# Jamy-L/Handheld-Multi-Frame-Super-Resolution

Measured on AMD Instinct MI355X. Metric: output Mpix/s for 12MP x 20-frame x2 SR burst; max-abs diff vs reference, higher is better.
Workload: dtype f32

## Files before the change

### handheld-multi-frame-super-resolution_amd/csrc/hhsr_robustness.hip

```cpp
#include "hhsr_common.h"

__device__ __forceinline__ double dodgson(double x) {
    const double a = fabs(x);
    if (a <= 0.5) return -2.0 * a * a + 1.0;
    if (a <= 1.5) return a * a - 5.0 / 2.0 * a + 1.5;
    return 0.0;
}

template <int NC>
__device__ __forceinline__ bool dodgson_sample(const float* __restrict__ LR, int lh, int lw, int y, int x, double fx,
                                               double fy, float out[NC]) {
    const double ly = ((double)y + fy + 0.5) / 2.0 - 0.5;
    const double lx = ((double)x + fx + 0.5) / 2.0 - 0.5;
    if (!(ly >= 0.0 && ly < (double)lh && lx >= 0.0 && lx < (double)lw)) return false;
    const int cy = (int)rint(ly), cx = (int)rint(lx);
    const size_t plane = (size_t)lh * lw;
    float b[NC];
#pragma unroll
    for (int c = 0; c < NC; ++c) b[c] = 0.f;
    double wacc = 0.0;
#pragma unroll
    for (int i = -1; i <= 1; ++i) {
        const int y_ = clampi(cy + i, 0, lh - 1);
        const double wy = dodgson((double)y_ - ly);
// ... 209 lines not shown
    const bool inb = dodgson_sample<3>(cm, lh, lw, y, x, (double)f.x, (double)f.y, cmu);
    if (!inb) cmu[0] = cmu[1] = cmu[2] = INFINITY;
    const size_t plane = (size_t)H * W, o = (size_t)y * W + x;
    double d_sq = 0.0;
#pragma unroll
    for (int c = 0; c < 3; ++c) {
        const float b = rmean[c * plane + o];
        const float dp = fabsf(b - cmu[c]);
        int id = 0;
        const double bb = 1000.0 * (double)b;
        if (isfinite(bb)) id = clampi((int)rint(bb), 0, ncurve - 1);
        const double d_t = difc[id];
        const float dp2f = dp * dp;
        const double dp2 = (double)dp2f;
        const double shrink = dp2 / (dp2 + d_t * d_t);
        d_sq += dp2 * shrink * shrink;
    }
    const float dsf = (float)d_sq, ssf = ssq[o];
    const float e = expf(-dsf / ssf);
    double v = (double)(S[(size_t)tiy * nx + tix] * e) - t;
    v = v > 0.0 ? v : 0.0;
    v = v < 1.0 ? v : 1.0;
    R[o] = (float)v;
}

constexpr int RF_T = 16;
constexpr int RF_BX = 32, RF_BY = 32;
constexpr int RF_WN = 11;

struct RobAxis {
    int fi;
    float h;
    bool lt, eq;
    bool ok;
};
__device__ __forceinline__ RobAxis rob_axis(float f) {
    const double fd = (double)f, fl = floor(fd), ff = fd - fl;
    RobAxis a;
    a.ok = fabs(fd) < 1.0e9;
    a.fi = a.ok ? (int)fl : 0;
    a.h = (float)(0.5 * ff);
    a.lt = ff < 0.5;
    a.eq = ff == 0.5;
    return a;
}
__device__ __forceinline__ bool rob_centre(const RobAxis& a, int p, int len, int& c, float& r) {
    const int n = p + a.fi, m = n >> 1, odd = n & 1;
    const bool up = odd && !a.lt && (!a.eq || (m & 1));
    c = m + (up ? 1 : 0);
    const float base = odd ? 0.25f + a.h : a.h - 0.25f;
    r = (up ? 1.0f : 0.0f) - base;
    return a.ok && (n >= 1 || (n == 0 && !a.lt)) && (n < 2 * len || (n == 2 * len && a.lt));
}
__device__ __forceinline__ void dodgson3(float r, int c, int len, float w[3]) {
    const float inner = fmaf(-2.0f * r, r, 1.0f);
    const float am = fabsf(r - 1.0f), ap = fabsf(r + 1.0f);
    const float om = fmaf(am, am, fmaf(-2.5f, am, 1.5f)), op = fmaf(ap, ap, fmaf(-2.5f, ap, 1.5f));
    w[0] = c - 1 >= 0 ? om : inner;
    w[1] = inner;
    w[2] = c + 1 <= len - 1 ? op : inner;
}

__device__ __forceinline__ void rob_row4(const float (*win)[RF_WN][RF_WN + 2], const RobAxis& ay, const RobAxis& ax,
                                         int wy0, int wx0, int y, int x0, int lh, int lw, const float rbk[4][3],
                                         const float d_t2[4][3], const float iss[4], float Sv, float tf, float out[4]) {
    int cy;
    float ry, wyv[3];
    const bool iny = rob_centre(ay, y, lh, cy, ry);
    dodgson3(ry, cy, lh, wyv);
    const int wi0 = cy - 1 - wy0;
    float cmu[4][3];
#pragma unroll
    for (int ph = 0; ph < 2; ++ph) {
        int cx;
        float rx;
        const bool inx = rob_centre(ax, x0 + ph, lw, cx, rx);
#pragma unroll
        for (int c = 0; c < 3; ++c) cmu[ph][c] = cmu[ph + 2][c] = INFINITY;
        if (iny && inx && cx >= 1 && cx + 2 <= lw - 1) {
            float wxv[3], w[3][3], wacc = 0.f;
            dodgson3(rx, cx, lw, wxv);
#pragma unroll
            for (int i = 0; i < 3; ++i)
#pragma unroll
                for (int j = 0; j < 3; ++j) {
                    w[i][j] = wyv[i] * wxv[j];
                    wacc += w[i][j];
                }
            const float iw = __builtin_amdgcn_rcpf(wacc);
            const int wj0 = cx - 1 - wx0;
#pragma unroll
            for (int c = 0; c < 3; ++c) {
                float g4[3][4];
#pragma unroll
                for (int i = 0; i < 3; ++i)
#pragma unroll
                    for (int j = 0; j < 4; ++j) g4[i][j] = win[c][wi0 + i][wj0 + j];
#pragma unroll
                for (int q = 0; q < 2; ++q) {
                    float b = 0.f;
#pragma unroll
                    for (int i = 0; i < 3; ++i)
#pragma unroll
                        for (int j = 0; j < 3; ++j) b = fmaf(g4[i][j + q], w[i][j], b);
                    cmu[ph + 2 * q][c] = b * iw;
                }
            }
        } else {
            int cx2;
            float rx2;
            const bool inx2 = rob_centre(ax, x0 + ph + 2, lw, cx2, rx2);
#pragma unroll
            for (int q = 0; q < 2; ++q) {
                const int cxq = q ? cx2 : cx;
                const float rxq = q ? rx2 : rx;
                if (iny && (q ? inx2 : inx)) {
                    float wxv[3], b0 = 0.f, b1 = 0.f, b2 = 0.f, wacc = 0.f;
                    dodgson3(rxq, cxq, lw, wxv);
                    const int wj0 = cxq - 1 - wx0;
#pragma unroll
                    for (int i = 0; i < 3; ++i) {
#pragma unroll
                        for (int j = 0; j < 3; ++j) {
                            const float w = wyv[i] * wxv[j];
                            b0 = fmaf(win[0][wi0 + i][wj0 + j], w, b0);
                            b1 = fmaf(win[1][wi0 + i][wj0 + j], w, b1);
                            b2 = fmaf(win[2][wi0 + i][wj0 + j], w, b2);
                            wacc += w;
                        }
                    }
                    const float iw = __builtin_amdgcn_rcpf(wacc);
                    cmu[ph + 2 * q][0] = b0 * iw;
                    cmu[ph + 2 * q][1] = b1 * iw;
                    cmu[ph + 2 * q][2] = b2 * iw;
                }
            }
        }
    }
#pragma unroll
    for (int k = 0; k < 4; ++k) {
        float d_sq = 0.f;
#pragma unroll
        for (int c = 0; c < 3; ++c) {
            const float dp = fabsf(rbk[k][c] - cmu[k][c]);
            const float dp2 = dp * dp;
            const float shrink = dp2 * __builtin_amdgcn_rcpf(dp2 + d_t2[k][c]);
            d_sq += dp2 * shrink * shrink;
        }
        const float e = __builtin_amdgcn_exp2f((-d_sq * iss[k]) * 1.44269504088896341f);
        out[k] = __builtin_amdgcn_fmed3f(Sv * e - tf, 0.f, 1.f);
    }
}

constexpr int ROB_GROUP = 4;
struct RobGroup {
    const float* cm[ROB_GROUP];
    const float2* flow[ROB_GROUP];
    const float* S[ROB_GROUP];
    float* R[ROB_GROUP];
    int n;
};

template <bool VEC, typename V, typename T>
__device__ __forceinline__ V rob_load4(const T* __restrict__ p, int x0, int W) {
    if constexpr (VEC) {
        return *reinterpret_cast<const V*>(p);
    } else {
        V v;
        v.x = x0 < W ? p[0] : T(0);
        v.y = x0 + 1 < W ? p[1] : T(0);
        v.z = x0 + 2 < W ? p[2] : T(0);
        v.w = x0 + 3 < W ? p[3] : T(0);
        return v;
    }
}
template <bool VEC>
__device__ __forceinline__ void rob_store4(float* __restrict__ p, const float out[4], int x0, int W) {
    if constexpr (VEC) {
        *reinterpret_cast<float4*>(p) = make_float4(out[0], out[1], out[2], out[3]);
    } else {
#pragma unroll
        for (int q = 0; q < 4; ++q)
            if (x0 + q < W) p[q] = out[q];
    }
}

template <bool VEC>
__global__ void __launch_bounds__(256) k_rob_frames_row4(RobGroup gq, int lh, int lw, const float* __restrict__ rmean,
                                                          const float* __restrict__ ssq,
                                                          const uint32_t* __restrict__ cidx, int ny, int nx, int ts,
                                                          const double* __restrict__ difc, double t, int H, int W,
                                                          double Mt2, float s1, float s2, int rows_lo, int rows_hi) {
    __shared__ float s_g[2][2][3][RF_WN][RF_WN + 2];
    __shared__ float4 s_tab[ROB_GROUP][2][2][2];
    const int lx4 = threadIdx.x & 7, ly_ = threadIdx.x >> 3;
    const int grp = lx4 >> 2, v = ly_ >> 4;
    const int bid = xcd_remap(blockIdx.y * gridDim.x + blockIdx.x, gridDim.x * gridDim.y);
    const int bxi = bid % gridDim.x, byi = bid / gridDim.x;
    const int x0 = bxi * RF_BX + 4 * lx4, y = byi * RF_BY + ly_;
    const size_t gplane = (size_t)lh * lw, plane = (size_t)H * W;
    const int tg = (ly_ & (RF_T - 1)) * 4 + (lx4 & 3);
    constexpr int WSZ = 3 * RF_WN * RF_WN, NST = (WSZ + 63) / 64;
    const bool live = x0 < W && y < H;
    const size_t o = live ? (size_t)y * W + x0 : 0;
    float4 rb4[3];
#pragma unroll
    for (int c = 0; c < 3; ++c) rb4[c] = rob_load4<VEC, float4>(rmean + c * plane + o, x0, W);
    const float4 ss4 = rob_load4<VEC, float4>(ssq + o, x0, W);
    const uint4 ci4 = rob_load4<VEC, uint4>(cidx + o, x0, W);
    const float rbk[4][3] = {{rb4[0].x, rb4[1].x, rb4[2].x}, {rb4[0].y, rb4[1].y, rb4[2].y},
                             {rb4[0].z, rb4[1].z, rb4[2].z}, {rb4[0].w, rb4[1].w, rb4[2].w}};
    const float ssk[4] = {ss4.x, ss4.y, ss4.z, ss4.w};
    const uint32_t cik[4] = {ci4.x, ci4.y, ci4.z, ci4.w};
    float d_t2[4][3], iss[4];
#pragma unroll
    for (int k = 0; k < 4; ++k) {
#pragma unroll
        for (int c = 0; c < 3; ++c) {
            const float d = (float)difc[(cik[k] >> (10 * c)) & 1023u];
            d_t2[k][c] = d * d;
        }
        iss[k] = __builtin_amdgcn_rcpf(ssk[k]);
    }
    if (threadIdx.x < gq.n * 4) {
        const int fr = threadIdx.x >> 2, vv = (threadIdx.x >> 1) & 1, gg = threadIdx.x & 1;
        const int tsx0 = bxi * RF_BX + gg * RF_T, tsy0 = byi * RF_BY + vv * RF_T;
        const size_t tl = (size_t)(min(tsy0, H - 1) / ts) * nx + min(tsx0, W - 1) / ts;
        const float2 f = gq.flow[fr][tl];
        const RobAxis ay = rob_axis(f.y), ax = rob_axis(f.x);
        int wy0, wx0;
        float r_;
        rob_centre(ay, tsy0, lh, wy0, r_);
        rob_centre(ax, tsx0, lw, wx0, r_);
        wy0 = clampi(wy0, -4, lh + 4) - 1;
        wx0 = clampi(wx0, -4, lw + 4) - 1;
        const int flags = (ay.lt ? 1 : 0) | (ay.eq ? 2 : 0) | (ay.ok ? 4 : 0) | (ax.lt ? 8 : 0) | (ax.eq ? 16 : 0) | (ax.ok ? 32 : 0);
        s_tab[fr][vv][gg][0] = make_float4(__int_as_float(ay.fi), ay.h, __int_as_float(wy0), __int_as_float(flags));
        float Sv;
        if (gq.S[fr]) {
            Sv = gq.S[fr][tl];
        } else {
            const int tiy = (int)(tl / nx), tix = (int)(tl - (size_t)tiy * nx);
            float mnx = INFINITY, mny = INFINITY, mxx = -INFINITY, mxy = -INFINITY;
            for (int i = -1; i <= 1; ++i)
                for (int j = -1; j <= 1; ++j) {
                    const int yy = tiy + i, xx = tix + j;
                    if (yy >= -rows_lo && yy < ny + rows_hi && xx >= 0 && xx < nx) {
                        const float2 q = gq.flow[fr][(ptrdiff_t)yy * nx + xx];
                        mxx = fmaxf(mxx, q.x); mxy = fmaxf(mxy, q.y);
                        mnx = fminf(mnx, q.x); mny = fminf(mny, q.y);
                    }
                }
            const float d0 = mxx - mnx, d1 = mxy - mny;
            const float m = d0 * d0 + d1 * d1;
            Sv = ((double)m > Mt2) ? s1 : s2;
        }
        s_tab[fr][vv][gg][1] = make_float4(__int_as_float(ax.fi), ax.h, __int_as_float(wx0), Sv);
    }
    __syncthreads();
    float st[NST];
    int fci[NST];
    unsigned fco[NST];
#pragma unroll
    for (int u = 0; u < NST; ++u) {
        const int p = tg + 64 * u;
        const int c = p / (RF_WN * RF_WN), q = p - c * (RF_WN * RF_WN);
        const int i = q / RF_WN, j = q - i * RF_WN;
        fci[u] = (i << 8) | j;
        fco[u] = (unsigned)c * (unsigned)gplane;
    }
    auto fetch = [&](int fr) {
        const float* __restrict__ cm = gq.cm[fr];
        const int wy0 = __float_as_int(s_tab[fr][v][grp][0].z), wx0 = __float_as_int(s_tab[fr][v][grp][1].z);
#pragma unroll
        for (int u = 0; u < NST; ++u) {
            const int p = tg + 64 * u;
            if (p < WSZ) {
                const int gy = clampi(wy0 + (fci[u] >> 8), 0, lh - 1), gx = clampi(wx0 + (fci[u] & 255), 0, lw - 1);
                const unsigned off = (fco[u] + (unsigned)(__mul24(gy, lw) + gx)) * 4u;
                st[u] = *reinterpret_cast<const float*>(reinterpret_cast<const char*>(cm) + off);
            }
        }
    };
    if (gq.n > 0) fetch(0);
    for (int fr = 0; fr < gq.n; ++fr) {
        const float4 t0 = s_tab[fr][v][grp][0], t1 = s_tab[fr][v][grp][1];
        const int flags = __float_as_int(t0.w);
        RobAxis ay, ax;
        ay.fi = __float_as_int(t0.x); ay.h = t0.y; ay.lt = flags & 1; ay.eq = flags & 2; ay.ok = flags & 4;
        ax.fi = __float_as_int(t1.x); ax.h = t1.y; ax.lt = flags & 8; ax.eq = flags & 16; ax.ok = flags & 32;
        const int wy0 = __float_as_int(t0.z), wx0 = __float_as_int(t1.z);
        const float Sv = t1.w;
        if (fr) __syncthreads();
#pragma unroll
        for (int u = 0; u < NST; ++u) {
            const int p = tg + 64 * u;
            if (p < WSZ) {
                const int c = p / (RF_WN * RF_WN), q = p - c * (RF_WN * RF_WN);
                const int i = q / RF_WN, j = q - i * RF_WN;
                s_g[grp][v][c][i][j] = st[u];
            }
        }
        __syncthreads();
        if (fr + 1 < gq.n) fetch(fr + 1);
        if (!live) continue;
        float out[4];
        rob_row4(s_g[grp][v], ay, ax, wy0, wx0, y, x0, lh, lw, rbk, d_t2, iss, Sv, (float)t, out);
        rob_store4<VEC>(gq.R[fr] + o, out, x0, W);
    }
}

static bool rob_grouped(int ts, const uint32_t* ref_curve_index, int ncurve) {
    return ts % RF_T == 0 && ref_curve_index && ncurve <= 1024;
}

static void rob_frames_launch(const float* const* comp_means, int n_frames, int lh, int lw, const float* ref_means,
                              const float* ref_sigma_sq, const uint32_t* ref_curve_index, const float* const* flows, int ny,
                              int nx, int ts, const float* const* S, double Mt, float s1, float s2, const double* diff_curve,
                              double t, float* const* R, int flow_rows_before, int flow_rows_after, hipStream_t stream) {
    const int H = 2 * lh, W = 2 * lw;
    bool vec = W % 4 == 0 && (((uintptr_t)ref_means | (uintptr_t)ref_sigma_sq | (uintptr_t)ref_curve_index) & 15) == 0;
    for (int n = 0; n < n_frames; ++n) vec = vec && ((uintptr_t)R[n] & 15) == 0;
    for (int n0 = 0; n0 < n_frames; n0 += ROB_GROUP) {
        RobGroup g;
        g.n = n_frames - n0 < ROB_GROUP ? n_frames - n0 : ROB_GROUP;
        for (int k = 0; k < ROB_GROUP; ++k) {
            const int n = n0 + (k < g.n ? k : 0);
            g.cm[k] = comp_means[n];
            g.flow[k] = reinterpret_cast<const float2*>(flows[n]);
            g.S[k] = S ? S[n] : nullptr;
            g.R[k] = R[n];
        }
        hipLaunchKernelGGL(vec ? k_rob_frames_row4<true> : k_rob_frames_row4<false>,
                           dim3(hhsr_cdiv(W, RF_BX), hhsr_cdiv(H, RF_BY)), dim3(256), 0, stream, g, lh, lw, ref_means,
                           ref_sigma_sq, ref_curve_index, ny, nx, ts, diff_curve, t, H, W, Mt * Mt, s1, s2, flow_rows_before,
                           flow_rows_after);
    }
}

extern "C" int hhsr_rob_frame(const float* comp_means, int lh, int lw, const float* ref_means,
                              const float* ref_sigma_sq, const uint32_t* ref_curve_index, const float* flow, int ny,
                              int nx, int ts, const float* S, const double* diff_curve, int ncurve, double t, float* R,
                              void* stream) {
    HHSR_ARG(comp_means && ref_means && ref_sigma_sq && flow && S && diff_curve && R);
    HHSR_ARG(lh > 0 && lw > 0 && ts > 0 && ncurve > 0);
    const int H = 2 * lh, W = 2 * lw;
    HHSR_ARG(ny * ts >= H && nx * ts >= W);
    if (rob_grouped(ts, ref_curve_index, ncurve))
        rob_frames_launch(&comp_means, 1, lh, lw, ref_means, ref_sigma_sq, ref_curve_index, &flow, ny, nx, ts, &S, 0.0, 0.f,
                          0.f, diff_curve, t, &R, 0, 0, (hipStream_t)stream);
    else
        hipLaunchKernelGGL(k_rob_frame, dim3(hhsr_cdiv(W, 64), hhsr_cdiv(H, 4)), dim3(256), 0, (hipStream_t)stream,
                           comp_means, lh, lw, ref_means, ref_sigma_sq, reinterpret_cast<const float2*>(flow), nx, ts,
                           S, diff_curve, ncurve, t, R, H, W);
    HHSR_LAUNCHED();
}

extern "C" int hhsr_rob_frames(const float* const* comp_means, int n_frames, int lh, int lw, const float* ref_means,
                               const float* ref_sigma_sq, const uint32_t* ref_curve_index, const float* const* flows,
                               int ny, int nx, int ts, const float* const* S, double Mt, float s1, float s2,
                               const double* diff_curve, int ncurve, double t, float* const* R, int flow_rows_before,
                               int flow_rows_after, void* stream) {
    HHSR_ARG(comp_means && flows && R && n_frames >= 0 && flow_rows_before >= 0 && flow_rows_after >= 0);
    for (int n = 0; n < n_frames; ++n) HHSR_ARG(comp_means[n] && flows[n] && (!S || S[n]) && R[n]);
    HHSR_ARG(ref_means && ref_sigma_sq && diff_curve && lh > 0 && lw > 0 && ts > 0 && ncurve > 0);
    const int H = 2 * lh, W = 2 * lw;
    HHSR_ARG(ny * ts >= H && nx * ts >= W);
    if (!rob_grouped(ts, ref_curve_index, ncurve)) {
        if (!S) {
            hhsr_set_error("hhsr_rob_frames: S = NULL (weights evaluated inside the kernel) needs the grouped kernel: "
                           "ts %% 16 == 0, packed curve indices");
            return -3;
        }
        for (int n = 0; n < n_frames; ++n) {
            const int rc = hhsr_rob_frame(comp_means[n], lh, lw, ref_means, ref_sigma_sq, ref_curve_index, flows[n], ny, nx,
                                          ts, S[n], diff_curve, ncurve, t, R[n], stream);
            if (rc) return rc;
        }
        return 0;
    }
    rob_frames_launch(comp_means, n_frames, lh, lw, ref_means, ref_sigma_sq, ref_curve_index, flows, ny, nx, ts, S, Mt, s1, s2,
                      diff_curve, t, R, flow_rows_before, flow_rows_after, (hipStream_t)stream);
    HHSR_LAUNCHED();
}

constexpr int LM_TX = 64, LM_TY = 16;

__global__ void __launch_bounds__(256) k_local_min5(const float* __restrict__ R, int H, int W,
                                                     float* __restrict__ r, float* __restrict__ acc) {
    __shared__ float s[LM_TY + 4][LM_TX + 4 + 1];
    __shared__ float s_row[LM_TY + 4][LM_TX + 1];
    const int x0 = blockIdx.x * LM_TX, y0 = blockIdx.y * LM_TY;
    for (int p = threadIdx.x; p < (LM_TY + 4) * (LM_TX + 4); p += 256) {
        const int i = p / (LM_TX + 4), j = p - i * (LM_TX + 4);
        s[i][j] = R[(size_t)clampi(y0 + i - 2, 0, H - 1) * W + clampi(x0 + j - 2, 0, W - 1)];
    }
    __syncthreads();
    for (int p = threadIdx.x; p < (LM_TY + 4) * LM_TX; p += 256) {
        const int i = p / LM_TX, j = p - i * LM_TX;
        float m = s[i][j];
#pragma unroll
        for (int k = 1; k < 5; ++k) m = fminf(m, s[i][j + k]);
        s_row[i][j] = m;
    }
    __syncthreads();
    for (int p = threadIdx.x; p < LM_TY * LM_TX; p += 256) {
        const int i = p / LM_TX, j = p - i * LM_TX;
        const int y = y0 + i, x = x0 + j;
        if (y < H && x < W) {
            float m = s_row[i][j];
#pragma unroll
            for (int k = 1; k < 5; ++k) m = fminf(m, s_row[i + k][j]);
            r[(size_t)y * W + x] = m;
            if (acc) acc[(size_t)y * W + x] += m;
        }
    }
}

extern "C" int hhsr_local_min5(const float* R, int H, int W, float* r, float* acc_r, void* stream) {
    HHSR_ARG(R && r && H > 0 && W > 0 && R != r);
    hipLaunchKernelGGL(k_local_min5, dim3(hhsr_cdiv(W, LM_TX), hhsr_cdiv(H, LM_TY)), dim3(256), 0,
                       (hipStream_t)stream, R, H, W, r, acc_r);
    HHSR_LAUNCHED();
}

struct RobSumFrames {
    const float* r[HHSR_MAX_FRAMES];
    int n;
};

__global__ void __launch_bounds__(256) k_rob_sum(RobSumFrames fr, size_t count, int load, double mfc, float m32, float below,
                                                  float above, double* __restrict__ sum64, float* __restrict__ mask32,
                                                  float* __restrict__ dec32) {
    const size_t i = (size_t)blockIdx.x * 256 + threadIdx.x;
    if (i >= count) return;
    double s = load ? sum64[i] : 0.0;
    for (int n = 0; n < fr.n; ++n) s += (double)fr.r[n][i];
    if (sum64) sum64[i] = s;
    float a = (float)s;
    if (mask32) mask32[i] = a;
    if (dec32) {
        if (s < mfc && a >= m32) a = below;
        if (s > mfc && a <= m32) a = above;
        dec32[i] = a;
    }
}

__global__ void __launch_bounds__(256) k_rob_sum_min5(RobSumFrames fr, int H, int W, int load, double mfc, float m32,
                                                       float below, float above, double* __restrict__ sum64,
                                                       float* __restrict__ mask32, float* __restrict__ dec32) {
    __shared__ float s[LM_TY + 4][LM_TX + 4 + 1];
    __shared__ float s_row[LM_TY + 4][LM_TX + 1];
    constexpr int NIN = ((LM_TY + 4) * (LM_TX + 4) + 255) / 256, NROW = (LM_TY + 4) * LM_TX / 256, NOUT = LM_TY * LM_TX / 256;
    const int x0 = blockIdx.x * LM_TX, y0 = blockIdx.y * LM_TY, tid = threadIdx.x;
    unsigned off[NIN];
#pragma unroll
    for (int u = 0; u < NIN; ++u) {
        const int p = tid + 256 * u, i = p / (LM_TX + 4), j = p - i * (LM_TX + 4);
        off[u] = (unsigned)(clampi(y0 + i - 2, 0, H - 1) * W + clampi(x0 + j - 2, 0, W - 1));
    }
    double acc[NOUT];
#pragma unroll
    for (int u = 0; u < NOUT; ++u) {
        const int p = tid + 256 * u, i = p / LM_TX, j = p - i * LM_TX;
        const bool live = y0 + i < H && x0 + j < W;
        acc[u] = (load && live) ? sum64[(size_t)(y0 + i) * W + x0 + j] : 0.0;
    }
    float pre[NIN];
    auto fetch = [&](int n) {
#pragma unroll
        for (int u = 0; u < NIN; ++u)
            if (tid + 256 * u < (LM_TY + 4) * (LM_TX + 4)) pre[u] = fr.r[n][off[u]];
    };
    if (fr.n > 0) fetch(0);
    for (int n = 0; n < fr.n; ++n) {
#pragma unroll
        for (int u = 0; u < NIN; ++u) {
            const int p = tid + 256 * u, i = p / (LM_TX + 4), j = p - i * (LM_TX + 4);
            if (p < (LM_TY + 4) * (LM_TX + 4)) s[i][j] = pre[u];
// ... 255 lines not shown
```

### handheld-multi-frame-super-resolution_amd/handheld_super_resolution/config.py

```python
from __future__ import annotations

import copy
from typing import Any, Mapping

__all__ = ["Config", "OmegaConf", "DEFAULTS", "default_config", "HIP_KNOBS", "hip_opt"]


class Config(dict):

    def __init__(self, data: Mapping | None = None, **kw):
        super().__init__()
        if data:
            for k, v in dict(data).items():
                self[k] = v
        for k, v in kw.items():
            self[k] = v

    @staticmethod
    def _wrap(v: Any) -> Any:
        if isinstance(v, Config):
            return v
        if isinstance(v, Mapping):
            return Config(v)
        if isinstance(v, tuple):
# ... 51 lines not shown
            raise AttributeError(k) from None

    def get(self, k, default=None):
        return self[k] if k in self else default

    def update(self, other=(), **kw):
        for k, v in dict(other, **kw).items():
            self[k] = v

    def copy(self):
        return Config(copy.deepcopy(dict(self)))

    def __deepcopy__(self, memo):
        return Config({k: copy.deepcopy(v, memo) for k, v in self.items()})


def _to_container(c):
    if isinstance(c, Mapping):
        return {k: _to_container(v) for k, v in c.items()}
    if isinstance(c, (list, tuple)):
        return [_to_container(v) for v in c]
    return c


def _merge_into(dst: Config, src: Mapping):
    for k, v in src.items():
        if isinstance(v, Mapping) and isinstance(dst.get(k), Mapping):
            _merge_into(dst[k], v)
        else:
            dst[k] = copy.deepcopy(v)


class OmegaConf:

    @staticmethod
    def create(obj=None):
        return Config(obj or {})

    @staticmethod
    def load(path):
        import yaml

        with open(path, "r") as f:
            return Config(yaml.safe_load(f) or {})

    @staticmethod
    def merge(*configs):
        out = Config()
        for c in configs:
            _merge_into(out, c)
        return out

    @staticmethod
    def to_container(cfg, resolve=True):
        return _to_container(cfg)

    @staticmethod
    def from_dotlist(items):
        import yaml

        out = Config()
        for it in items:
            key, _, val = it.partition("=")
            node = out
            parts = key.split(".")
            for p in parts[:-1]:
                if p not in node:
                    node[p] = {}
                node = node[p]
            node[parts[-1]] = yaml.safe_load(val)
        return out


DEFAULTS = {
    "scale": 1,
    "mode": "bayer",
    "debug": False,
    "verbose": 1,
    "grey_method": "FFT",
    "noise_model": {"alpha": None, "beta": None},
    "block_matching": {
        "tuning": {
            "factors": [1, 2, 4, 4],
            "tile_size": "SNR_based",
            "tile_size_factors": [1, 1, 1, 0.5],
            "search_radii": [1, 4, 4, 4],
            "metrics": ["L1", "L2", "L2", "L2"],
            "flow_upscale_mode": "nearest",
        }
    },
    "ica": {"tuning": {"n_iter": 3, "sigma_blur": 0}},
    "robustness": {
        "enabled": True,
        "save_mask": True,
        "tuning": {"t": 0.12, "s1": 2, "s2": 12, "Mt": 0.8},
    },
    "merging": {
        "kernel": "steerable",
        "selection_law": "linear",
        "tuning": {
            "k_detail": "SNR_based",
            "k_denoise": "SNR_based",
            "D_th": "SNR_based",
            "D_tr": "SNR_based",
            "k_stretch": 4,
            "k_shrink": 2,
        },
    },
    "postprocessing": {
        "enabled": True,
        "do_color_correction": False,
        "do_gamma_correction": True,
        "do_tonemapping": False,
        "sharpening": {"enabled": True, "amount": 1.5, "radius": 3},
        "do_devignetting": False,
    },
    "accumulated_robustness_denoiser": {
        "median": {"enabled": False, "radius_max": 3, "max_frame_count": 8},
        "gauss": {"enabled": False, "sigma_max": 1.5, "max_frame_count": 8},
        "merge": {"enabled": False, "rad_max": 2, "max_multiplier": 8, "max_frame_count": 2},
    },
    "compat": {
        "ica64_row_bug": True,
    },
}


def default_config(**overrides) -> Config:
    cfg = Config(copy.deepcopy(DEFAULTS))
    if overrides:
        _merge_into(cfg, overrides)
    return cfg


HIP_KNOBS = {
    "graph": True,
    "batch": True,
    "fused_merge": True,
    "fused_align": True,
    "weight_fp64": False,
    "merge_kernel": "auto",
    "strategy": "rows",
    "stage_frames": 0,
    "chunk": None,
    "streams": None,
    "merge_chain": None,
    "merge_link_after": None,
    "host_chunk_sizes": None,
    "inject_flows": None,
    "raw_norm": None,
    "max_flow": None,
    "align_cost": None,
}


def hip_opt(config, name):
    default = HIP_KNOBS[name]
    hip = config.get("hip", None) if hasattr(config, "get") else None
    return default if hip is None else hip.get(name, default)
```

### handheld-multi-frame-super-resolution_amd/handheld_super_resolution/super_resolution.py

```python
import atexit
import os
import threading
import time

import numpy as np
import torch

from . import _lib
from .config import hip_opt
from .utils_image import compute_grey_images, compute_grey_images_batch
from .utils import divide, add, getTime, timer
from .alignment import init_alignment, build_gaussian_pyramids, align_batch, can_align_batch
from .params import sanitize_config, update_snr_config
from .robustness import (init_robustness, compute_robustness, compute_robustness_group, noise_curves_to_device, RobustnessSum,
                         ref_planes, upscale_warp_stats, mono_sigma_sq)
from .kernels import estimate_kernels, frame_stats, frame_stats_batch
from .merge import merge, merge_ref, merge_burst, can_fuse_acc_r, merge_fusions


def denoiser_enabled(config, store=True):
    den = config.accumulated_robustness_denoiser
    if "enabled" in den:
        return bool(den.enabled)
    on = bool(den.median.enabled or den.gauss.enabled or den.merge.enabled)
    if store:
        den.enabled = on
    return on


def accumulation(config):
    denoiser_on = denoiser_enabled(config)
    return denoiser_on, denoiser_on or bool(config.robustness.save_mask)


def main_plan(config, shape, n_comp, denoiser_on, accumulate_r):
    fused_merge = bool(hip_opt(config, "fused_merge"))
    quiet = not (config.verbose >= 1 or bool(config.debug))
    fused = fused_merge and not denoiser_on
    den_fused = fused_merge and denoiser_on and can_fuse_acc_r(config) and n_comp > 0 and quiet
    batch = (fused and quiet) or den_fused
    fuse_acc, fuse_min = merge_fusions(config, shape, n_comp, accumulate_r and not den_fused, denoiser_on)
    return fused, batch, fused and fuse_acc, batch and fuse_min, den_fused


def _device():
    if not torch.cuda.is_available():
        raise RuntimeError("handheld_super_resolution (MI355X build): no HIP device is visible; this package has no "
                           "CPU path (the NumPy oracle under oracle/ is test infrastructure only)")
    return torch.device("cuda", torch.cuda.current_device())


ROB_GROUP = 4


def front_groups(k, batch, given, robustness, mono, batchable):
    whole = k >= 2 and batch and ((given == k and robustness and not mono) or (given == 0 and batchable))
    return [k] if whole else [1] * k


def _tensors(x):
    if torch.is_tensor(x):
        yield x
    elif isinstance(x, (tuple, list)):
        for y in x:
            yield from _tensors(y)


DEFAULT_STREAMS = 2
LARGE_FRAME = 40_000_000
_stream_pool = {}


class _Staged:
    __slots__ = ("tensor", "event")

    def __init__(self, tensor, event):
        self.tensor, self.event = tensor, event


_upload_streams = {}


_LATE_FORK = os.environ.get("HHSR_LATE_FORK") is not None


class BurstPipeline:

    def __init__(self, config, device=None):
        self.config = config
        self.device = device or _device()
        self.mono = config.mode != "bayer"
        self.cfa = [[int(v) for v in row] for row in config.exif.cfa_pattern]
        self.wb = [float(v) for v in config.exif.white_balance]
        self.curves = noise_curves_to_device(config.noise_model.std_curve, config.noise_model.diff_curve, self.device)
        self.grey_method = config.grey_method
        self.ref = None
        self._streams = _stream_pool.setdefault(self.device.index, [])
        self._inject_flows = hip_opt(config, "inject_flows")
        self._raw_norm = hip_opt(config, "raw_norm")
        self.flow_rows = (0, 0)
        self.ref_wait = True
        self._batch = bool(hip_opt(config, "batch")) and (self.mono or self.grey_method == "FFT") and config.verbose < 2

    def _ingest(self, img):
        staged = isinstance(img, _Staged)
        if staged:
            if img.event is not None:
                cur = torch.cuda.current_stream(self.device)
                cur.wait_event(img.event)
                img.tensor.record_stream(cur)
            img = img.tensor
        t = img if torch.is_tensor(img) else torch.as_tensor(img)
        if t.dtype.is_floating_point:
            return _lib.f32c(t, self.device)
        if (t.is_cuda and not staged) or self._raw_norm is None:
            raise ValueError("integer frames are sensor counts: give config.hip.raw_norm = {black_levels, white_level} "
                             "(host arrays), or pass normalised float frames")
        from .utils_dng import normalize_burst, normalize_packed, packed_width

        width = packed_width(self._raw_norm, t)
        if width is not None:
            return normalize_packed(t, width, self._raw_norm["packing"], self._raw_norm["black_levels"],
                                    self._raw_norm["white_level"], self.wb, self.cfa, device=self.device)
        return normalize_burst(t, self._raw_norm["black_levels"], self._raw_norm["white_level"], self.wb, self.cfa,
                               device=self.device)

    def prefetch(self, imgs):
        out, stream = [], None
        for img in imgs:
            t = img if torch.is_tensor(img) else (torch.as_tensor(img) if isinstance(img, np.ndarray) else None)
            if t is None or t.is_cuda or not t.is_pinned():
                out.append(img)
                continue
            if stream is None:
                stream = _upload_streams.get(self.device.index)
                if stream is None:
                    from .graph import shared_streams

                    stream = _upload_streams[self.device.index] = shared_streams(self.device)[1]
            if t.dtype == torch.float64:
                t = t.to(torch.float32).pin_memory()
            with torch.cuda.stream(stream):
                d = t.contiguous().to(self.device, non_blocking=True)
                ev = torch.cuda.Event()
                ev.record(stream)
            self._last_upload = ev
            out.append(_Staged(d, ev))
        return out

    def uploads_done(self):
        ev = getattr(self, "_last_upload", None)
        if ev is not None:
            ev.synchronize()
            self._last_upload = None

    def _timed(self, func, level, start_s=None, end_s=None):
        return timer(func, self.config.verbose >= level, start_s, end_s)

    def init_ref(self, ref_img, alignment=True, robustness=True):
        with torch.cuda.device(self.device):
            return self._init_ref(ref_img, alignment, robustness)

    def _init_ref(self, ref_img, alignment, robustness):
        cfg = self.config
        main = torch.cuda.current_stream(self.device)
        self._entry = torch.cuda.Event()
        self._entry.record(main)
        self._entry_fresh = True
        self.ref = self._ingest(ref_img)
        self.align_state = self.grey_ref = None
        if alignment:
            sanitize_config(cfg, tuple(self.ref.shape))
            grey = self.ref if self.mono else self._timed(
                compute_grey_images, 3, end_s="- Ref grey image estimated by {}".format(self.grey_method))(
                self.ref, self.grey_method)
            self.align_state = self._timed(init_alignment, 2, "\nInitializing alignment", "Alignment initialized (Total)")(
                grey, cfg)
            self.grey_ref = grey
        self._align_ready = torch.cuda.Event()
        self._align_ready.record(main)
        self.ref_means = self.ref_vars = self.ref_covs = self.ref_sigma_sq = None
        if robustness and cfg.robustness.enabled and self.mono:
            m, v, self.ref_covs = self._timed(frame_stats, 2, "\nEstimating ref image local stats + kernels",
                                              "Local stats + kernels estimated (Total)")(
                self.ref, self.cfa, self.wb, cfg, want_vars=True)
            self.ref_means, self.ref_vars = upscale_warp_stats(m), upscale_warp_stats(v)
            self.ref_sigma_sq = mono_sigma_sq(self.ref_means, self.ref_vars, self.curves[0])
        elif robustness and cfg.robustness.enabled:
            m, v, self.ref_covs = self._timed(frame_stats, 2, "\nEstimating ref image local stats + kernels",
                                              "Local stats + kernels estimated (Total)")(
                self.ref, self.cfa, self.wb, cfg, want_vars=True)
            self.ref_means, self.ref_sigma_sq = ref_planes(m, v, self.curves[0])
            self.ref_vars = None
        elif robustness:
            self.ref_means, self.ref_vars = init_robustness(self.ref, self.cfa, self.wb, cfg)
            self.ref_covs = estimate_kernels(self.ref, cfg)
        self._ref_ready = torch.cuda.Event()
        self._ref_ready.record(main)
        return self

    def flow_grid(self):
        lvl0 = self.align_state[0][-1]
        ts = int(self.config.block_matching.tuning.tile_size)
        return lvl0.shape[0] // ts, lvl0.shape[1] // ts

    def align_frames(self, comp_imgs, n_streams=None):
        with torch.cuda.device(self.device):
            comp_imgs = self.prefetch([comp_imgs[i] for i in range(len(comp_imgs))])
            chunks = self._chunks(len(comp_imgs), n_streams)
            out = self._on_streams(len(chunks), n_streams, False,
                                   lambda ci, wait: self._grouped(comp_imgs, wait, chunks[ci], None, stats=False))
            return [f for chunk in out for f in chunk]

    def _grouped(self, imgs, wait_ref, indices, flows, stats=True):
        fl = [None if flows is None else flows[i] for i in indices]
        groups = front_groups(len(indices), self._batch, sum(f is not None for f in fl), bool(self.config.robustness.enabled),
                              self.mono, can_align_batch(self.config))
        out, i0 = [], 0
        for k in groups:
            out += self._front_group([imgs[i] for i in indices[i0:i0 + k]], wait_ref, fl[i0:i0 + k], stats)
            i0 += k
        return out

    def _front_group(self, imgs, wait_ref, flows, stats=True):
        cfg = self.config
        raws = [self._ingest(img) for img in imgs]
        if flows[0] is not None:
            flows = [_lib.f32c(f, self.device) for f in flows]
        else:
            greys = raws if self.mono else self._timed(
                compute_grey_images_batch, 3, end_s="- grey images estimated by {}".format(self.grey_method))(raws, self.grey_method)
            pyramids = build_gaussian_pyramids(greys, cfg.block_matching.tuning.factors)
            if wait_ref is not None:
                torch.cuda.current_stream(self.device).wait_event(self._align_ready)
            st = self.align_state
            flows = self._timed(align_batch, 2, "\nBeginning alignment", "Image aligned (Total)")(
                st[0], st[5], pyramids, cfg, st[3], st[4])
        if not stats:
            return flows
        if not cfg.robustness.enabled:
            est = self._timed(estimate_kernels, 2, "\nEstimating kernels", "Kernels estimated (Total)")
            return [(raw, f, est(raw, cfg), None) for raw, f in zip(raws, flows)]
        stat = self._timed(frame_stats if self.mono else frame_stats_batch, 2, "\nEstimating kernels + guide statistics",
                           "Kernels + guide statistics estimated (Total)")
        sts = [stat(raw, self.cfa, self.wb, cfg) for raw in raws] if self.mono else stat(raws, self.cfa, self.wb, cfg)
        return [(raw, f, st[2], st[0]) for raw, f, st in zip(raws, flows, sts)]

    def _robustness(self, fronts, accumulate_r=None, fuse_local_min=False):
        cfg = self.config
        if not cfg.robustness.enabled or len(fronts) == 1 or self.mono:
            rob = self._timed(compute_robustness, 2, "\nEstimating robustness", "Robustness estimated (Total)")
            return [(raw, flow, covs,
                     rob(raw, self.ref_means, self.ref_vars, flow, self.cfa, self.wb, self.curves, cfg,
                                        accumulate_into=accumulate_r, ref_sigma_sq=self.ref_sigma_sq, comp_means=means,
                                        fuse_local_min=fuse_local_min and cfg.robustness.enabled,
                                        flow_rows=self.flow_rows))
                    for raw, flow, covs, means in fronts]
        rs = compute_robustness_group([f[0] for f in fronts], self.ref_means, [f[1] for f in fronts], self.curves, cfg,
                                      self.ref_sigma_sq, [f[3] for f in fronts], accumulate_into=accumulate_r,
                                      fuse_local_min=fuse_local_min, flow_rows=self.flow_rows)
        return [(f[0], f[1], f[2], r) for f, r in zip(fronts, rs)]

    def process_frame(self, img, accumulate_r=None, wait_ref=None, fuse_local_min=False, index=None, flow=None):
        if flow is None and self._inject_flows is not None and index is not None:
            flow = self._inject_flows[index]
        fronts = self._front_group([img], wait_ref, [flow])
        if wait_ref is not None:
            torch.cuda.current_stream(self.device).wait_event(wait_ref)
        return self._robustness(fronts, accumulate_r, fuse_local_min)[0]

    def process_frames(self, comp_imgs, accumulate_r=None, n_streams=None, fuse_local_min=False, flows=None):
        with torch.cuda.device(self.device):
            n = len(comp_imgs)
            comp_imgs = self.prefetch(comp_imgs)
            chunks = self._chunks(n, n_streams)
            if flows is None:
                flows = self._inject_flows

            def work(ci, wait):
                fronts = self._grouped(comp_imgs, wait, chunks[ci], flows)
                if wait is not None:
                    torch.cuda.current_stream(self.device).wait_event(wait)
                return self._robustness(fronts, accumulate_r if wait is None else None, fuse_local_min)

            out = self._on_streams(len(chunks), n_streams, accumulate_r is not None, work)
            return [f for chunk in out for f in chunk]

    def _chunks(self, n, n_streams=None):
        streams = self._n_streams(n_streams)
        size = self._chunk_size()
        n_chunks = min(n, streams * -(-n // (streams * size))) if n else 0
        chunks, i = [], 0
        for c in range(n_chunks):
            k = n // n_chunks + (1 if c < n % n_chunks else 0)
            chunks.append(list(range(i, i + k)))
            i += k
        return chunks

    def _chunk_size(self):
        chunk = hip_opt(self.config, "chunk")
        return max(1, min(ROB_GROUP if chunk is None else int(chunk), _lib.MAX_BATCH))

    def _n_streams(self, n_streams):
        if n_streams is None:
            n_streams = hip_opt(self.config, "streams")
        if n_streams is None:
            n_streams = 1 if self.ref is not None and self.ref.numel() >= LARGE_FRAME else DEFAULT_STREAMS
        return max(1, int(n_streams))

    def _on_streams(self, n, n_streams, serial, work):
        n_streams = self._n_streams(n_streams)
        early = bool(self.ref_wait and getattr(self, "_entry_fresh", False) and n_streams > 1 and not serial and n >= 1
                     and not _LATE_FORK)
        self._entry_fresh = False
        if not early and (n_streams <= 1 or serial or n < 2):
            return [work(i, None) for i in range(n)]
        main = torch.cuda.current_stream(self.device)
        if len(self._streams) < n_streams:
            self._streams += [torch.cuda.Stream(self.device) for _ in range(n_streams - len(self._streams))]
        pool = self._streams[:n_streams]
        entry = torch.cuda.Event()
        entry.record(main)
        for s in pool:
            s.wait_event(self._entry if early else entry)
        results = []
        for i in range(n):
            s = pool[i % n_streams]
            with torch.cuda.stream(s):
                f = work(i, entry if early else (self._ref_ready if self.ref_wait else None))
            for t in _tensors(f):
                t.record_stream(main)
            results.append(f)
        for s in pool:
            main.wait_stream(s)
        return results

    def output_size(self):
        s = self.config.scale
        H, W = self.ref.shape
        return round(s * H), round(s * W)


_main_runners = []
_main_runners_lock = threading.Lock()


def _drop_host_runners():
    while _main_runners:
        _, _, runner = _main_runners.pop()
        runner.close()


atexit.register(_drop_host_runners)


def _host_runner(config, device):
    from .graph import ConfigWatch, HostBurstRunner

    with _main_runners_lock:
        for k, (cfg, watch, runner) in enumerate(_main_runners):
            if cfg is config and runner.device == device:
                _main_runners.append(_main_runners.pop(k))
                if watch.changed(config):
                    _main_runners.pop()
                    break
                return runner
        watch = ConfigWatch()
        watch.changed(config)
        runner = HostBurstRunner(config, device)
        _main_runners.append((config, watch, runner))
        while len(_main_runners) > 2:
            _main_runners.pop(0)[2].close()
        return runner


def main(ref_img, comp_imgs, config, *, _no_runner=False):
    if not _no_runner and torch.cuda.is_available():
        from .graph import HostBurstRunner

        denoiser_enabled(config)
        if HostBurstRunner.usable(config, ref_img, comp_imgs):
            return _host_runner(config, _device()).call_cloned(ref_img, comp_imgs)
    verbose = config.verbose >= 1
    debug_mode = bool(config.debug)
    debug_dict = {"robustness": [], "flow": []}
    denoiser_on, accumulate_r = accumulation(config)

    if verbose:
        torch.cuda.synchronize()
        t1 = time.perf_counter()
        print("\nProcessing reference image ---------\n")
    pipe = BurstPipeline(config).init_ref(ref_img)
    dev = pipe.device
    H, W = pipe.ref.shape
    sH, sW = pipe.output_size()
    fused, batch, fuse_acc, fuse_min, den_fused = main_plan(config, (H, W), len(comp_imgs), denoiser_on, accumulate_r)
    acc_sum = RobustnessSum((H, W), dev) if denoiser_on else None
    accumulated_r = torch.zeros((H, W), dtype=torch.float32, device=dev) if (accumulate_r and not denoiser_on) else None
    num = torch.empty((sH, sW, 3), dtype=torch.float32, device=dev)
    den = None
    if den_fused:
        den = torch.empty_like(num)
    elif not fused:
        num.zero_()
        den = torch.zeros_like(num)
    if verbose:
        torch.cuda.synchronize()
        getTime(t1, "\nRef Img processed (Total)")

    frames = []
    n_images = len(comp_imgs)
    if batch:
        frames = pipe.process_frames([comp_imgs[i] for i in range(n_images)], None if fuse_acc else accumulated_r,
                                     fuse_local_min=fuse_min)
        if den_fused:
            acc_sum.add_many([f[3] for f in frames], unfiltered=fuse_min)
        n_images = 0
    for im_id in range(n_images):
        if verbose:
            torch.cuda.synchronize()
            print("\nProcessing image {} ---------\n".format(im_id + 1))
            im_time = time.perf_counter()
        raw, flow, covs, r = pipe.process_frame(comp_imgs[im_id], None if fuse_acc else accumulated_r, index=im_id)
        if acc_sum is not None:
            acc_sum.add(r)
        if fused:
            frames.append((raw, flow, covs, r))
        else:
            pipe._timed(merge, 2, "\nAccumulating Image", "Image accumulated (Total)")(raw, flow, covs, r, num, den, pipe.cfa,
                                                                                          config)
        if debug_mode:
            debug_dict["flow"].append(flow.cpu().numpy())
            debug_dict["robustness"].append(r.cpu().numpy())
        if verbose:
            torch.cuda.synchronize()
            getTime(im_time, "\nImage processed (Total)")

    ref_covs = pipe.ref_covs
    if fused:
        pipe._timed(merge_burst, 2, "\nAccumulating all frames + ref Img + normalising", "Burst merged (Total)")(
            frames, pipe.ref, ref_covs, num, None, pipe.cfa, config, do_ref=True, divide=True,
            acc_r=accumulated_r if fuse_acc else None, local_min=fuse_min)
    else:
        if den_fused:
            merge_burst(frames, None, None, num, den, pipe.cfa, config, do_ref=False, divide=False, store_den=True,
                        local_min=fuse_min)
        dec = acc_sum.for_decisions(config.accumulated_robustness_denoiser.merge.max_frame_count) if denoiser_on else None
        if den_fused:
            merge_ref(pipe.ref, ref_covs, num, den, pipe.cfa, config, dec, divide=True, fast=True)
        else:
            pipe._timed(merge_ref, 2, "\nAccumulating ref Img", "Ref Img accumulated (Total)")(
                pipe.ref, ref_covs, num, den, pipe.cfa, config, dec)
            pipe._timed(divide, 2, end_s="\n------------------------\nImage normalized (Total)")(num, den)
    if verbose:
        torch.cuda.synchronize()
        s = "\nTotal ellapsed time : "
        print(s, " " * (50 - len(s)), ": ", round((time.perf_counter() - t1), 2), "seconds")
    if accumulate_r:
        debug_dict["accumulated robustness"] = acc_sum.mask() if denoiser_on else accumulated_r
    pipe.uploads_done()
    return num, debug_dict


def prepare_config(config, ref_raw, alpha=None, beta=None, cfa_pattern=None, white_balance=None, iso=100,
                   std_curve=None, diff_curve=None, shape=None):
    from .synthetic import noise_curves

    if config.noise_model.get("alpha", None) is not None:
        alpha, beta = config.noise_model.alpha, config.noise_model.beta
    if alpha is None or beta is None:
        raise ValueError("noise model (alpha, beta) missing: give it in config.noise_model or in the burst")
    config.noise_model.update({"alpha": float(alpha), "beta": float(beta)})
    if std_curve is None or diff_curve is None:
        std_curve, diff_curve = noise_curves(float(alpha), float(beta))
    brightness = float(ref_raw.mean()) if torch.is_tensor(ref_raw) else float(np.mean(ref_raw))
    id_noise = min(max(round(1000 * brightness), 0), len(std_curve) - 1)
    SNR = brightness / float(std_curve[id_noise])
    if config.verbose >= 1:
        print(" ", 10 * "-")
        print("|ISO : {}".format(iso))
        print("|Image brightness : {:.2f}".format(brightness))
        print("|expected noise std : {:.2e}".format(float(std_curve[id_noise])))
        print("|Estimated SNR : {:.2f}".format(SNR))
    update_snr_config(config, SNR)
    sanitize_config(config, tuple(shape if shape is not None else ref_raw.shape))
# ... 133 lines not shown
```

Before: 6392.

## Batch robustness over all frames per stream instead of per chunk

```diff
diff --git a/handheld-multi-frame-super-resolution_amd/csrc/hhsr_robustness.hip b/handheld-multi-frame-super-resolution_amd/csrc/hhsr_robustness.hip
--- a/handheld-multi-frame-super-resolution_amd/csrc/hhsr_robustness.hip
+++ b/handheld-multi-frame-super-resolution_amd/csrc/hhsr_robustness.hip
@@ -385,14 +385,15 @@
     }
 }
 
-constexpr int ROB_GROUP = 4;
+constexpr int ROB_CAP = HHSR_MAX_FRAMES;
 struct RobGroup {
-    const float* cm[ROB_GROUP];
-    const float2* flow[ROB_GROUP];
-    const float* S[ROB_GROUP];
-    float* R[ROB_GROUP];
+    const float* cm[ROB_CAP];
+    const float2* flow[ROB_CAP];
+    const float* S[ROB_CAP];
+    float* R[ROB_CAP];
     int n;
 };
+static_assert(sizeof(RobGroup) + 128 <= 4096, "RobGroup is a by-value kernel argument: 4 KB of kernarg segment");
 
 template <bool VEC, typename V, typename T>
 __device__ __forceinline__ V rob_load4(const T* __restrict__ p, int x0, int W) {
@@ -425,7 +426,7 @@
                                                           const double* __restrict__ difc, double t, int H, int W,
                                                           double Mt2, float s1, float s2, int rows_lo, int rows_hi) {
     __shared__ float s_g[2][2][3][RF_WN][RF_WN + 2];
-    __shared__ float4 s_tab[ROB_GROUP][2][2][2];
+    __shared__ float4 s_tab[ROB_CAP][2][2][2];
     const int lx4 = threadIdx.x & 7, ly_ = threadIdx.x >> 3;
     const int grp = lx4 >> 2, v = ly_ >> 4;
     const int bid = xcd_remap(blockIdx.y * gridDim.x + blockIdx.x, gridDim.x * gridDim.y);
@@ -455,8 +456,8 @@
         }
         iss[k] = __builtin_amdgcn_rcpf(ssk[k]);
     }
-    if (threadIdx.x < gq.n * 4) {
-        const int fr = threadIdx.x >> 2, vv = (threadIdx.x >> 1) & 1, gg = threadIdx.x & 1;
+    for (int it = threadIdx.x; it < gq.n * 4; it += 256) {
+        const int fr = it >> 2, vv = (it >> 1) & 1, gg = it & 1;
         const int tsx0 = bxi * RF_BX + gg * RF_T, tsy0 = byi * RF_BY + vv * RF_T;
         const size_t tl = (size_t)(min(tsy0, H - 1) / ts) * nx + min(tsx0, W - 1) / ts;
         const float2 f = gq.flow[fr][tl];
@@ -554,10 +555,10 @@
     const int H = 2 * lh, W = 2 * lw;
     bool vec = W % 4 == 0 && (((uintptr_t)ref_means | (uintptr_t)ref_sigma_sq | (uintptr_t)ref_curve_index) & 15) == 0;
     for (int n = 0; n < n_frames; ++n) vec = vec && ((uintptr_t)R[n] & 15) == 0;
-    for (int n0 = 0; n0 < n_frames; n0 += ROB_GROUP) {
+    for (int n0 = 0; n0 < n_frames; n0 += ROB_CAP) {
         RobGroup g;
-        g.n = n_frames - n0 < ROB_GROUP ? n_frames - n0 : ROB_GROUP;
-        for (int k = 0; k < ROB_GROUP; ++k) {
+        g.n = n_frames - n0 < ROB_CAP ? n_frames - n0 : ROB_CAP;
+        for (int k = 0; k < ROB_CAP; ++k) {
             const int n = n0 + (k < g.n ? k : 0);
             g.cm[k] = comp_means[n];
             g.flow[k] = reinterpret_cast<const float2*>(flows[n]);
diff --git a/handheld-multi-frame-super-resolution_amd/handheld_super_resolution/config.py b/handheld-multi-frame-super-resolution_amd/handheld_super_resolution/config.py
--- a/handheld-multi-frame-super-resolution_amd/handheld_super_resolution/config.py
+++ b/handheld-multi-frame-super-resolution_amd/handheld_super_resolution/config.py
@@ -227,9 +227,12 @@
     "max_flow": None,
     "align_cost": None,
 }
+HIP_PLACEMENTS = {
+    "rob_launch": "stream",
+}
 
 
 def hip_opt(config, name):
-    default = HIP_KNOBS[name]
+    default = HIP_PLACEMENTS[name] if name in HIP_PLACEMENTS else HIP_KNOBS[name]
     hip = config.get("hip", None) if hasattr(config, "get") else None
     return default if hip is None else hip.get(name, default)
diff --git a/handheld-multi-frame-super-resolution_amd/handheld_super_resolution/super_resolution.py b/handheld-multi-frame-super-resolution_amd/handheld_super_resolution/super_resolution.py
--- a/handheld-multi-frame-super-resolution_amd/handheld_super_resolution/super_resolution.py
+++ b/handheld-multi-frame-super-resolution_amd/handheld_super_resolution/super_resolution.py
@@ -50,7 +50,8 @@
     return torch.device("cuda", torch.cuda.current_device())
 
 
-ROB_GROUP = 4
+DEFAULT_CHUNK = 4
+ROB_LAUNCHES = ("stream", "burst", "chunk")
 
 
 def front_groups(k, batch, given, robustness, mono, batchable):
@@ -277,14 +278,30 @@
             if flows is None:
                 flows = self._inject_flows
 
-            def work(ci, wait):
-                fronts = self._grouped(comp_imgs, wait, chunks[ci], flows)
+            launch = self._rob_launch(accumulate_r)
+
+            def rob(fronts, wait):
                 if wait is not None:
                     torch.cuda.current_stream(self.device).wait_event(wait)
                 return self._robustness(fronts, accumulate_r if wait is None else None, fuse_local_min)
 
-            out = self._on_streams(len(chunks), n_streams, accumulate_r is not None, work)
-            return [f for chunk in out for f in chunk]
+            def work(ci, wait):
+                fronts = self._grouped(comp_imgs, wait, chunks[ci], flows)
+                return rob(fronts, wait) if launch == "chunk" else fronts
+
+            def tail(outs, wait):
+                done = iter(rob([f for chunk in outs for f in chunk], wait)) if outs else None
+                return [[next(done) for _ in chunk] for chunk in outs]
+
+            out = self._on_streams(len(chunks), n_streams, accumulate_r is not None, work, tail if launch == "stream" else None)
+            out = [f for chunk in out for f in chunk]
+            return rob(out, None) if launch == "burst" and out else out
+
+    def _rob_launch(self, accumulate_r=None):
+        launch = hip_opt(self.config, "rob_launch")
+        if launch not in ROB_LAUNCHES:
+            raise ValueError(f"config.hip.rob_launch: {launch!r} is not one of {ROB_LAUNCHES}")
+        return "chunk" if (accumulate_r is not None or self.mono or not self.config.robustness.enabled) else launch
 
     def _chunks(self, n, n_streams=None):
         streams = self._n_streams(n_streams)
@@ -299,7 +316,7 @@
 
     def _chunk_size(self):
         chunk = hip_opt(self.config, "chunk")
-        return max(1, min(ROB_GROUP if chunk is None else int(chunk), _lib.MAX_BATCH))
+        return max(1, min(DEFAULT_CHUNK if chunk is None else int(chunk), _lib.MAX_BATCH))
 
     def _n_streams(self, n_streams):
         if n_streams is None:
@@ -308,13 +325,14 @@
             n_streams = 1 if self.ref is not None and self.ref.numel() >= LARGE_FRAME else DEFAULT_STREAMS
         return max(1, int(n_streams))
 
-    def _on_streams(self, n, n_streams, serial, work):
+    def _on_streams(self, n, n_streams, serial, work, tail=None):
         n_streams = self._n_streams(n_streams)
         early = bool(self.ref_wait and getattr(self, "_entry_fresh", False) and n_streams > 1 and not serial and n >= 1
                      and not _LATE_FORK)
         self._entry_fresh = False
         if not early and (n_streams <= 1 or serial or n < 2):
-            return [work(i, None) for i in range(n)]
+            out = [work(i, None) for i in range(n)]
+            return out if tail is None else tail(out, None)
         main = torch.cuda.current_stream(self.device)
         if len(self._streams) < n_streams:
             self._streams += [torch.cuda.Stream(self.device) for _ in range(n_streams - len(self._streams))]
@@ -324,13 +342,17 @@
         for s in pool:
             s.wait_event(self._entry if early else entry)
         results = []
+        wait = entry if early else (self._ref_ready if self.ref_wait else None)
         for i in range(n):
             s = pool[i % n_streams]
             with torch.cuda.stream(s):
-                f = work(i, entry if early else (self._ref_ready if self.ref_wait else None))
-            for t in _tensors(f):
-                t.record_stream(main)
-            results.append(f)
+                results.append(work(i, wait))
+                if tail is not None and i + n_streams >= n:
+                    mine = range(i % n_streams, n, n_streams)
+                    for j, f in zip(mine, tail([results[j] for j in mine], wait)):
+                        results[j] = f
+        for t in _tensors(results):
+            t.record_stream(main)
         for s in pool:
             main.wait_stream(s)
         return results
```

Result: no change. 6429, median of 2 (+0.6%).
